# voxelmorph/voxelmorph

Measured on NVIDIA H100. Metric: vol-pairs/sec (3D 160x192x224 VxmDense int_steps=7 train step, NCC+Grad, Adam), higher is better.
Workload: dtype bf16 (conv operands) / f32 (accumulate, warp, VecInt, losses)

## Files before the change

voxelmorph_b200/csrc/conv3d_tc_s.cu:

```cuda
#include <stdlib.h>
#include <string.h>

#include "tc_common.cuh"

namespace vxm {
namespace tcs {

using namespace vxm::tc;

constexpr int WT = 32, WUSE = 30;
constexpr int MAXSLOT = 16;
constexpr int NLOADER = 128, NTHREADS = 384, NGRP = 2;

struct ConvSArgs {
  const __nv_bfloat16* xa; const __nv_bfloat16* xb;
  const __nv_bfloat16* wpk; const float* bias;
  void* out; const __nv_bfloat16* mask;
  void* out2; int csplit;
  int B, D, H, W, Ca, Cb, up, upd, Cout, out_mode;
  float slope;
  int tiles_h, tiles_w, dchunk, nchunks, nitems, nslot;
  uint32_t wbytes;
  const float* acc_in; void* out_lo;
  int tma_mask, tc0[2];
  int opitch;
  alignas(64) CUtensorMap tm[2];
};

__host__ __device__ inline uint32_t swz(uint32_t off, uint32_t width) {
  return off ^ (((off >> 7) & (width / 16 - 1)) << 4);
}
__device__ __forceinline__ uint64_t make_desc_kmajor_swz(uint32_t saddr, uint32_t width) {
  uint64_t d = 0;
  d |= (uint64_t)((saddr >> 4) & 0x3FFF);
  d |= (uint64_t)1 << 16;
  d |= (uint64_t)(((8u * width) >> 4) & 0x3FFF) << 32;
  return d | desc_swizzle(width);
}

template <int KD, int G0, int G1, int COUT, int HT, bool ACC, int EPI, bool OP = false, int PD = 0>
__global__ void __launch_bounds__(NTHREADS, 1) conv_tcs_kernel(const __grid_constant__ ConvSArgs a) {
  static_assert(PD == 0 || (KD == 3 && EPI != 0 && !ACC && !OP), "polyphase forms: 3-D, specialised epilogue");
  static_assert(PD != 1 || G1 > 0, "the polyphase forward merges channel group 0 and keeps group 1");
  static_assert(PD != 2 || (G1 == 0 && COUT == 32 && HT == 8 && EPI == 2), "the coarse dgrad: 32 -> 32 channels, 8-row tiles");
  constexpr int SROWS = (HT + 2) * WT;
  constexpr int NH = PD == 2 ? 1 : HT / 4;
  constexpr int NEVEN = (HT + 3) / 2;
  constexpr int W0 = G0 * 2, W1 = G1 * 2;
  constexpr int NC8 = (G0 + G1) / 8;
  constexpr uint32_t SLAB0 = SROWS * W0, SLAB1 = SROWS * W1;
  constexpr int NN = 3 * COUT;
  extern __shared__ __align__(1024) uint8_t smem[];
  const bool halfk = (a.Ca + a.Cb == 8);
  constexpr uint32_t slab_bytes = SLAB0 + SLAB1;
  const int NSLOT = a.nslot;
  uint8_t* s_w = smem;
  uint8_t* s_slab = smem + ((a.wbytes + 1023u) & ~1023u);
  float* s_stage = reinterpret_cast<float*>(s_slab + NSLOT * slab_bytes);
  uint64_t* bars = reinterpret_cast<uint64_t*>(s_stage + NGRP * ACC_STAGE_FLOATS);
  uint64_t* full = bars;
  uint64_t* empty = bars + MAXSLOT;
  uint64_t* wbar = empty + MAXSLOT;

  const int warp = threadIdx.x >> 5, lane = threadIdx.x & 31;

  const bool tma0 = a.tma_mask & 1, tma1 = (a.tma_mask & 2) != 0;
  const bool all_tma = tma0 && (G1 == 0 || tma1);
  if (threadIdx.x == 0) {
    for (int i = 0; i < NSLOT; ++i) { mbar_init(&full[i], all_tma ? 1 : NLOADER); mbar_init(&empty[i], 4 * NGRP); }
    mbar_init(wbar, 1);
    fence_barrier_init();
  }
  __syncthreads();

  if (threadIdx.x == 0) {
    mbar_expect_tx(wbar, a.wbytes);
    for (uint32_t off = 0; off < a.wbytes; off += 16384u) {
      uint32_t n = a.wbytes - off < 16384u ? a.wbytes - off : 16384u;
      bulk_g2s(s_w + off, reinterpret_cast<const uint8_t*>(a.wpk) + off, n, wbar);
    }
  }
  const int HW_tiles = a.tiles_h * a.tiles_w;
  const int Dout = PD == 2 ? a.D >> 1 : a.D;

  if (warp >= 8) {
    const int lt = threadIdx.x - 8 * 32;
    uint32_t slot = 0, lphase = 1;
    const int Da = a.upd ? a.D >> 1 : a.D, Ha = a.up ? a.H >> 1 : a.H, Wa = a.up ? a.W >> 1 : a.W;
    const int nca8 = a.Ca >> 3;
    constexpr int nchunk = NC8 * SROWS;
    constexpr int KMAX = (nchunk + NLOADER - 1) / NLOADER;
    if (lt == 0) {
      if (tma0) tma_prefetch_desc(&a.tm[0]);
      if (tma1) tma_prefetch_desc(&a.tm[1]);
    }
    const uint32_t tma_bytes = (tma0 ? SLAB0 : 0u) + (tma1 ? SLAB1 : 0u);
    for (int item = blockIdx.x; item < a.nitems && !(all_tma && lt != 0); item += gridDim.x) {
      const int wt = item % a.tiles_w, ht = (item / a.tiles_w) % a.tiles_h;
      const int ch = (item / HW_tiles) % a.nchunks, b = item / (HW_tiles * a.nchunks);
      const int h0 = ht * HT, w0 = wt * WUSE, d0 = ch * a.dchunk, d1 = min(d0 + a.dchunk, Dout);
      const int s_begin = PD == 2 ? 2 * d0 - 1 : (KD == 3 ? d0 - 1 : d0), s_end = PD == 2 ? 2 * d1 + 1 : (KD == 3 ? d1 + 1 : d1);
      int soff[KMAX];
      uint32_t doff[KMAX];
#pragma unroll
      for (int k = 0; k < KMAX; ++k) {
        const int id = lt + k * NLOADER;
        soff[k] = -1;
        doff[k] = 0;
        if (id < nchunk) {
          const int c8 = id % NC8, row = id / NC8;
          const int r = row >> 5, c = row & 31;
          const int h = h0 - 1 + r, w = w0 - 1 + c;
          const int srow = PD == 2 ? ((r & 1) ? NEVEN + (r >> 1) : (r >> 1)) * WT + c : row;
          doff[k] = c8 < G0 / 8 ? swz((uint32_t)srow * W0 + (uint32_t)c8 * 16u, W0)
                                : SLAB0 + swz((uint32_t)row * W1 + (uint32_t)(c8 - G0 / 8) * 16u, W1 ? W1 : 32);
          if (c8 < G0 / 8 ? tma0 : tma1) soff[k] = -2;
          else if (h >= 0 && h < a.H && w >= 0 && w < a.W && !(halfk && c8 > 0)) {
            if (c8 < nca8) soff[k] = (((a.up ? h >> 1 : h) * Wa + (a.up ? w >> 1 : w)) * a.Ca + c8 * 8) << 1;
            else soff[k] = (((h * a.W + w) * a.Cb + (c8 - nca8) * 8) << 1) | 1;
          }
        }
      }
      for (int ds = s_begin; ds < s_end; ++ds) {
        mbar_wait(&empty[slot], lphase);
        uint8_t* slab = s_slab + (size_t)slot * slab_bytes;
        const bool dok = ds >= 0 && ds < a.D;
        const __nv_bfloat16* baseA = a.xa ? a.xa + (((size_t)b * Da + (dok ? (a.upd ? ds >> 1 : ds) : 0)) * Ha * Wa) * a.Ca : nullptr;
        const __nv_bfloat16* baseB = a.xb ? a.xb + (((size_t)b * a.D + (dok ? ds : 0)) * a.H * a.W) * a.Cb : nullptr;
        const __nv_bfloat16* dummy = a.xa ? a.xa : a.xb;
        if (lt == 0 && tma_bytes) {
          if (all_tma) mbar_expect_tx(&full[slot], tma_bytes);
          else mbar_expect_tx_noarrive(&full[slot], tma_bytes);
          if (tma0) tma_load_5d(slab, &a.tm[0], a.tc0[0], w0 - 1, h0 - 1, ds, b, &full[slot]);
          if (tma1) tma_load_5d(slab + SLAB0, &a.tm[1], a.tc0[1], w0 - 1, h0 - 1, ds, b, &full[slot]);
        }
        if (!all_tma) {
#pragma unroll
          for (int k = 0; k < KMAX; ++k) {
            if (lt + k * NLOADER < nchunk && soff[k] != -2) {
              const bool ok = dok && soff[k] >= 0;
              const __nv_bfloat16* src = ok ? ((soff[k] & 1) ? baseB : baseA) + (soff[k] >> 1) : dummy;
              cp_async16(slab + doff[k], src, ok ? 16u : 0u);
            }
          }
          cp_async_arrive_noinc(&full[slot]);
        }
        if (++slot == (uint32_t)NSLOT) { slot = 0; lphase ^= 1; }
      }
    }
  } else {
    const int grp = warp >> 2;
    const int wq = warp & 3;
    float* stage = s_stage + grp * ACC_STAGE_FLOATS;
    const int nbar = 1 + grp;
    constexpr int NSUB = NN > 96 ? 2 : 1;
    constexpr int NF = 2 / NSUB;
    constexpr int NCH = NSUB == 1 ? COUT / 16 : (COUT + 31) / 32;
    const int trow0 = NSUB == 1 ? wq : (wq & 1);
    auto chan = [&](int i) { return NSUB == 1 ? 16 * i : 32 * i + 16 * (wq >> 1); };
    const uint32_t slab_u32 = smem_u32(s_slab), w_u32 = smem_u32(s_w);
    constexpr uint32_t WSTEP = (uint32_t)NN * (W0 + W1);
    mbar_wait(wbar, 0);
    const uint64_t bdesc0 = make_desc_kmajor_swz(w_u32, W0);
    const uint64_t bdesc1 = make_desc_kmajor_swz(w_u32 + NN * W0, W1 ? W1 : 32);
    uint32_t cnt_base = 0, ecnt = 0, wcur = 0;
    auto observe = [&](uint32_t upto) {
      for (; wcur <= upto; ++wcur) mbar_wait(&full[wcur % NSLOT], (wcur / NSLOT) & 1);
    };
    constexpr int NKD = PD == 2 ? 4 : KD;
    auto mma = [&](uint32_t hslot, int hb, int sub, float (&acc)[NF][NN / 2], int par) {
      uint64_t adesc0_kd[NKD], adesc1_kd[NKD];
      uint32_t sl = hslot;
#pragma unroll
      for (int kd = 0; kd < NKD; ++kd) {
        adesc0_kd[kd] = make_desc_kmajor_swz(slab_u32 + sl * slab_bytes, W0);
        adesc1_kd[kd] = make_desc_kmajor_swz(slab_u32 + sl * slab_bytes + SLAB0, W1 ? W1 : 32);
        if (++sl == (uint32_t)NSLOT) sl = 0;
      }
      wg_fence();
#pragma unroll
      for (int kd = 0; kd < NKD; ++kd) {
#pragma unroll
        for (int kh = 0; kh < (PD == 2 ? 4 : 3); ++kh) {
          const int st = kd * (PD == 2 ? 4 : 3) + kh;
#pragma unroll
          for (int k = 0; k < (G0 + G1) / 16; ++k) {
            const bool g0 = k < G0 / 16;
            if (PD == 1 && g0 && kd == 2) continue;
            const int kk = g0 ? k : k - G0 / 16;
            const uint32_t wr = g0 ? W0 : W1;
            uint64_t abase = g0 ? adesc0_kd[kd] : adesc1_kd[kd];
            uint32_t wst = st * WSTEP;
            if (PD == 1 && g0 && par) {
              abase = adesc0_kd[kd + 1 < NKD ? kd + 1 : kd];
              wst = kd == 0 ? 9 * WSTEP + kh * NN * W0 : (6 + kh) * WSTEP;
            }
            const int r0 = PD == 2 ? ((kh & 1) ? NEVEN : 0) + (kh >> 1) : hb * 4 + kh;
            const uint64_t adesc = abase + (uint64_t)((r0 * WT * wr + kk * 32) >> 4);
            const uint64_t bdesc = (g0 ? bdesc0 : bdesc1) + (uint64_t)((wst + kk * 32) >> 4);
#pragma unroll
            for (int f = 0; f < NF; ++f)
              Wgmma<NN, 0, 0>::mma(acc[f], adesc + (uint64_t)(((sub + f) * 2 * WT * wr) >> 4), bdesc, (st | k) ? 1u : 0u);
          }
        }
      }
      wg_commit();
      wg_wait<0>();
    };
    auto readout = [&](float (&acc)[NF][NN / 2], int c, uint32_t (&r)[16]) {
      if constexpr (NSUB == 1) acc_row16(acc[0], acc[NF - 1], c, stage, nbar, r);
      else acc_half_row16(acc[0], c, COUT - (c % COUT) < 32 ? 16 : 32, stage, nbar, r);
    };
    auto combine = [&](float (&acc)[NF][NN / 2], int i, float (&v)[16]) {
      const int cb = NSUB == 1 ? 16 * i : 32 * i;
      uint32_t r[16];
      readout(acc, cb, r);
#pragma unroll
      for (int c = 0; c < 16; ++c) v[c] = __shfl_up_sync(0xffffffffu, __uint_as_float(r[c]), 1);
      readout(acc, COUT + cb, r);
#pragma unroll
      for (int c = 0; c < 16; ++c) v[c] += __uint_as_float(r[c]);
      readout(acc, 2 * COUT + cb, r);
#pragma unroll
      for (int c = 0; c < 16; ++c) v[c] += __shfl_down_sync(0xffffffffu, __uint_as_float(r[c]), 1);
    };
    auto release = [&](int nd) {
      if (KD == 3) {
        const uint32_t last = PD == 2 ? 2u * nd : (uint32_t)nd;
        observe(cnt_base + last + 1u);
        if (lane == 0) {
          mbar_arrive(&empty[(cnt_base + last) % NSLOT]);
          mbar_arrive(&empty[(cnt_base + last + 1) % NSLOT]);
        }
        cnt_base += last + 2;
      } else {
        cnt_base += nd;
      }
    };
    if constexpr (EPI != 0) {
      const float slope = a.slope;
      const int c1 = (EPI == 3 && a.out2) ? a.csplit : COUT;
      const int Ho = PD == 2 ? a.H >> 1 : a.H, Wo = PD == 2 ? a.W >> 1 : a.W;
      const size_t HWp = (size_t)Ho * Wo;
      for (int item = blockIdx.x; item < a.nitems; item += gridDim.x) {
        const int wt = item % a.tiles_w, ht = (item / a.tiles_w) % a.tiles_h;
        const int ch = (item / HW_tiles) % a.nchunks, b = item / (HW_tiles * a.nchunks);
        const int w = wt * WUSE - 1 + lane, d0 = ch * a.dchunk, d1 = min(d0 + a.dchunk, Dout);
        const int nd = d1 - d0;
        const bool wok = lane >= 1 && lane <= WUSE && w < a.W && (PD != 2 || (lane & 1));
        bool ok[NH][NSUB];
        size_t vx[NH][NSUB];
#pragma unroll
        for (int hb = 0; hb < NH; ++hb) {
#pragma unroll
          for (int sub = 0; sub < NSUB; ++sub) {
            const int h = PD == 2 ? ht * (HT / 2) + trow0 : ht * HT + hb * 4 + trow0 + 2 * sub;
            ok[hb][sub] = wok && h < Ho;
            vx[hb][sub] = (((size_t)b * Dout + d0) * Ho + h) * Wo + (PD == 2 ? w >> 1 : w);
          }
        }
        for (int j = 0; j < nd; ++j) {
          const uint32_t js = PD == 2 ? 2u * j : (uint32_t)j;
          observe(cnt_base + js + (PD == 2 ? 3u : (KD == 3 ? 2u : 0u)));
          const uint32_t hslot = (cnt_base + js) % NSLOT;
#pragma unroll
          for (int hb = 0; hb < NH; ++hb) {
            const bool mine = (int)(ecnt++ % NGRP) == grp;
            size_t voxs[NSUB];
#pragma unroll
            for (int sub = 0; sub < NSUB; ++sub) {
              voxs[sub] = vx[hb][sub];
              vx[hb][sub] += HWp;
            }
            if (!mine) continue;
#pragma unroll
            for (int sub = 0; sub < NSUB; ++sub) {
              const size_t vox = voxs[sub];
              const bool valid = ok[hb][sub];
              [[maybe_unused]] uint32_t mreg[EPI == 2 ? NCH : 1][8];
              if constexpr (EPI == 2) {
#pragma unroll
                for (int i = 0; i < NCH; ++i)
                  if (valid && chan(i) < COUT) ld_global_nc_v8(a.mask + vox * (OP ? a.opitch : COUT) + chan(i), mreg[i]);
              }
              float acc[NF][NN / 2];
              mma(hslot, hb, sub, acc, (d0 + j) & 1);
#pragma unroll
              for (int i = 0; i < NCH; ++i) {
                const int c0 = chan(i);
                float v[16];
                combine(acc, i, v);
                if (NSUB > 1 && c0 >= COUT) continue;
                if constexpr (PD == 2) {
#pragma unroll
                  for (int c = 0; c < 16; ++c) v[c] += __shfl_down_sync(0xffffffffu, v[c], 1);
                }
                if constexpr (EPI == 1) {
#pragma unroll
                  for (int c = 0; c < 16; ++c) {
                    const float x = v[c] + (a.bias ? __ldg(a.bias + c0 + c) : 0.f);
                    v[c] = fmaxf(x, x * slope);
                  }
                } else if constexpr (EPI == 2) {
#pragma unroll
                  for (int e = 0; e < 8; ++e) {
                    const uint32_t mw = mreg[i][e];
                    if (mw & 0x8000u) v[2 * e] *= slope;
                    if (mw & 0x80000000u) v[2 * e + 1] *= slope;
                  }
                }
                if (valid) {
                  __nv_bfloat16* dst = (EPI == 3 && c0 >= c1) ? reinterpret_cast<__nv_bfloat16*>(a.out2) + vox * (COUT - c1) + (c0 - c1)
                                                              : reinterpret_cast<__nv_bfloat16*>(a.out) + vox * (OP ? a.opitch : c1) + c0;
                  st_global_v8(dst, pack_bf16x2(v[0], v[1]), pack_bf16x2(v[2], v[3]), pack_bf16x2(v[4], v[5]), pack_bf16x2(v[6], v[7]),
                               pack_bf16x2(v[8], v[9]), pack_bf16x2(v[10], v[11]), pack_bf16x2(v[12], v[13]), pack_bf16x2(v[14], v[15]));
                }
              }
            }
          }
          if (lane == 0) {
            mbar_arrive(&empty[hslot]);
            if (PD == 2) mbar_arrive(&empty[(hslot + 1) % NSLOT]);
          }
        }
        release(nd);
      }
    } else {
    const size_t HWp = (size_t)a.H * a.W;
    auto bias_at = [&](int c) -> float { return a.bias ? __ldg(a.bias + c) : 0.f; };
    for (int item = blockIdx.x; item < a.nitems; item += gridDim.x) {
      const int wt = item % a.tiles_w, ht = (item / a.tiles_w) % a.tiles_h;
      const int ch = (item / HW_tiles) % a.nchunks, b = item / (HW_tiles * a.nchunks);
      const int w = wt * WUSE - 1 + lane, d0 = ch * a.dchunk, d1 = min(d0 + a.dchunk, a.D);
      const int nd = d1 - d0;
      for (int j = 0; j < nd; ++j) {
        const int d = d0 + j;
        observe(cnt_base + (uint32_t)j + (KD == 3 ? 2u : 0u));
        const uint32_t hslot = (cnt_base + j) % NSLOT;
#pragma unroll
        for (int hb = 0; hb < NH; ++hb) {
        if ((int)(ecnt++ % NGRP) != grp) continue;
#pragma unroll
        for (int sub = 0; sub < NSUB; ++sub) {
        const int h = ht * HT + hb * 4 + trow0 + 2 * sub;
        const bool valid = lane >= 1 && lane <= WUSE && h < a.H && w < a.W;
        const size_t vox = (((size_t)b * a.D + d) * a.H + h) * a.W + w;
        constexpr bool PREF = NSUB == 1;
        [[maybe_unused]] uint4 mreg[PREF ? NCH : 1][2];
        if (PREF && a.mask && valid) {
#pragma unroll
          for (int i = 0; i < NCH; ++i)
#pragma unroll
            for (int q = 0; q < 2; ++q)
              if (chan(i) + 8 * q < a.Cout)
                mreg[i][q] = __ldg(reinterpret_cast<const uint4*>(a.mask + vox * (OP ? a.opitch : a.Cout) + chan(i)) + q);
        }
        const int c1 = a.out2 ? a.csplit : a.Cout;
        float acc[NF][NN / 2];
        mma(hslot, hb, sub, acc, 0);
#pragma unroll
        for (int i = 0; i < NCH; ++i) {
          const int c0 = chan(i);
          [[maybe_unused]] float4 ain[ACC ? 4 : 1];
          if constexpr (ACC && !OP && PREF) {
            if (a.acc_in && valid && c0 < COUT) {
              const float4* ap = reinterpret_cast<const float4*>(a.acc_in + vox * COUT + c0);
#pragma unroll
              for (int q = 0; q < 4; ++q) ain[q] = __ldg(ap + q);
            }
          }
          float v[16];
          combine(acc, i, v);
          if (NSUB > 1 && c0 >= COUT) continue;
          bool handled = false;
          if constexpr (ACC) {
            if (a.acc_in && valid) {
              if constexpr (OP || !PREF) {
                const float4* ap = reinterpret_cast<const float4*>(a.acc_in + vox * COUT + c0);
#pragma unroll
                for (int q = 0; q < 4; ++q) ain[q] = __ldg(ap + q);
              }
#pragma unroll
              for (int q = 0; q < 4; ++q) { v[4 * q] += ain[q].x; v[4 * q + 1] += ain[q].y; v[4 * q + 2] += ain[q].z; v[4 * q + 3] += ain[q].w; }
            }
            if (a.out_mode == 2) {
              handled = true;
              if (valid) {
                float4* op = reinterpret_cast<float4*>(reinterpret_cast<float*>(a.out) + vox * COUT + c0);
#pragma unroll
                for (int q = 0; q < 4; ++q) op[q] = make_float4(v[4 * q], v[4 * q + 1], v[4 * q + 2], v[4 * q + 3]);
              }
            } else if (a.out_mode == 3) {
              handled = true;
              if (valid && c0 < a.Cout) {
#pragma unroll
                for (int q = 0; q < 16; q += 8) {
                  if (c0 + q < a.Cout) {
                    uint32_t hi[4], lo[4];
#pragma unroll
                    for (int e = 0; e < 8; e += 2) {
                      float x0 = v[q + e] + bias_at(c0 + q + e), x1 = v[q + e + 1] + bias_at(c0 + q + e + 1);
                      if (a.slope >= 0.f) { x0 = x0 >= 0.f ? x0 : x0 * a.slope; x1 = x1 >= 0.f ? x1 : x1 * a.slope; }
                      const __nv_bfloat16 h0 = __float2bfloat16_rn(x0), h1 = __float2bfloat16_rn(x1);
                      hi[e >> 1] = (uint32_t)__bfloat16_as_ushort(h0) | ((uint32_t)__bfloat16_as_ushort(h1) << 16);
                      lo[e >> 1] = pack_bf16x2(x0 - __bfloat162float(h0), x1 - __bfloat162float(h1));
                    }
                    const size_t o = vox * (OP ? a.opitch : a.Cout) + c0 + q;
                    *reinterpret_cast<uint4*>(reinterpret_cast<__nv_bfloat16*>(a.out) + o) = make_uint4(hi[0], hi[1], hi[2], hi[3]);
                    *reinterpret_cast<uint4*>(reinterpret_cast<__nv_bfloat16*>(a.out_lo) + o) = make_uint4(lo[0], lo[1], lo[2], lo[3]);
                  }
                }
              }
            }
          }
          if (!handled && valid && c0 < a.Cout) {
            if (a.out_mode == 0) {
#pragma unroll
              for (int q = 0; q < 16; q += 8) {
                if (c0 + q < a.Cout) {
                  float x[8];
#pragma unroll
                  for (int e = 0; e < 8; ++e) x[e] = v[q + e] + bias_at(c0 + q + e);
                  if (a.mask) {
                    uint4 m4;
                    if constexpr (PREF) m4 = mreg[i][q / 8];
                    else m4 = __ldg(reinterpret_cast<const uint4*>(a.mask + vox * (OP ? a.opitch : a.Cout) + c0) + q / 8);
                    const __nv_bfloat16* mb = reinterpret_cast<const __nv_bfloat16*>(&m4);
#pragma unroll
                    for (int e = 0; e < 8; ++e) if (__bfloat162float(mb[e]) < 0.f) x[e] *= a.slope;
                  } else if (a.slope >= 0.f) {
#pragma unroll
                    for (int e = 0; e < 8; ++e) x[e] = x[e] >= 0.f ? x[e] : x[e] * a.slope;
                  }
                  const int cg = c0 + q;
                  __nv_bfloat16* oo = cg < c1 ? reinterpret_cast<__nv_bfloat16*>(a.out) + vox * (OP ? a.opitch : c1) + cg
                                              : reinterpret_cast<__nv_bfloat16*>(a.out2) + vox * (a.Cout - c1) + (cg - c1);
                  *reinterpret_cast<uint4*>(oo) = make_uint4(pack_bf16x2(x[0], x[1]), pack_bf16x2(x[2], x[3]), pack_bf16x2(x[4], x[5]), pack_bf16x2(x[6], x[7]));
                }
              }
            } else {
              float* o = reinterpret_cast<float*>(a.out);
#pragma unroll
              for (int c = 0; c < 16; ++c) {
                if (c0 + c < a.Cout) {
                  float x = v[c] + bias_at(c0 + c);
                  if (a.slope >= 0.f) x = x >= 0.f ? x : x * a.slope;
                  o[(((size_t)b * a.Cout + c0 + c) * a.D + d) * HWp + (size_t)h * a.W + w] = x;
                }
              }
            }
          }
        }
        }
        }
        if (lane == 0) mbar_arrive(&empty[hslot]);
      }
      release(nd);
    }
    }
  }
}

__global__ void pack_weights_s_kernel(const float* __restrict__ w, __nv_bfloat16* __restrict__ out, int Cout, int Cin, int KD, int COUT,
                                      int NN, int G0, int G1, int transposed) {
  const int T = KD * 9;
  const int CG = G0 + G1;
  const int total = KD * 3 * NN * CG;
  for (int i = blockIdx.x * blockDim.x + threadIdx.x; i < total; i += gridDim.x * blockDim.x) {
    const int ci = i % CG, n = (i / CG) % NN, st = i / (CG * NN);
    const int kd = st / 3, kh = st % 3, g = n / COUT, co = n % COUT;
    const int tap = (kd * 3 + kh) * 3 + g;
    float v = 0.f;
    if (!transposed) {
      if (co < Cout && ci < Cin) v = w[((size_t)co * Cin + ci) * T + tap];
    } else {
      if (co < Cin && ci < Cout) v = w[((size_t)ci * Cin + co) * T + (T - 1 - tap)];
    }
    const uint32_t W0 = G0 * 2, W1 = G1 * 2;
    uint32_t off;
    if (ci < G0) off = swz((uint32_t)n * W0 + (uint32_t)ci * 2u, W0);
    else off = (uint32_t)NN * W0 + swz((uint32_t)n * W1 + (uint32_t)(ci - G0) * 2u, W1);
    out[((size_t)st * NN * (W0 + W1) + off) / 2] = __float2bfloat16_rn(v);
  }
}

struct PackDesc {
  const float* w;
  __nv_bfloat16* out;
  int Cout, Cin, KD, COUT, NN, G0, G1, transposed;
  int begin, count;
  int fold;
  int n0, nb, k0, kb;
  int poly;
};
__global__ void pack_weights_multi_kernel(const PackDesc* __restrict__ descs, int ndesc, int total) {
  for (int gi = blockIdx.x * blockDim.x + threadIdx.x; gi < total; gi += gridDim.x * blockDim.x) {
    int lo = 0, hi = ndesc - 1;
    while (lo < hi) {
      const int mid = (lo + hi + 1) >> 1;
      if (descs[mid].begin <= gi) lo = mid; else hi = mid - 1;
    }
    const PackDesc d = descs[lo];
    const int i = gi - d.begin;
    const int T = d.KD * 9, CG = d.G0 + d.G1;
    const int base = d.KD * 3 * d.NN * CG;
    const bool extra = d.poly == 1 && i >= base;
    const int ie = i - base;
    const int ci = extra ? ie % d.G0 : i % CG, n = extra ? (ie / d.G0) % d.NN : (i / CG) % d.NN;
    const int st = extra ? ie / (d.G0 * d.NN) : i / (CG * d.NN);
    const int kd = extra ? 0 : (d.poly == 2 ? st >> 2 : st / 3), kh = extra ? st : (d.poly == 2 ? st & 3 : st % 3);
    const int g = n / d.COUT, co = n % d.COUT;
    const int tap = (kd * 3 + kh) * 3 + g;
    float v = 0.f;
    if (d.poly) {
      if (co < d.nb && ci < d.kb) {
        int t0 = kd, t1 = kd, u0 = kh, u1 = kh;
        if (d.poly == 1 && ci < d.G0) t1 = extra ? 1 : (kd == 1 ? 2 : kd);
        if (d.poly == 2) {
          t0 = kd > 0 ? kd - 1 : 0; t1 = kd < 2 ? kd : 2;
          u0 = kh > 0 ? kh - 1 : 0; u1 = kh < 2 ? kh : 2;
        }
        for (int t = t0; t <= t1; ++t)
          for (int u = u0; u <= u1; ++u) {
            const int tp = (t * 3 + u) * 3 + g;
            v += !d.transposed ? d.w[((size_t)(d.n0 + co) * d.Cin + d.k0 + ci) * 27 + tp]
                               : d.w[((size_t)(d.k0 + ci) * d.Cin + d.n0 + co) * 27 + (26 - tp)];
          }
      }
    } else if (d.fold) {
      const int fk = ci / d.fold, c = ci % d.fold;
      const int tap3 = (fk * 3 + kh) * 3 + g;
      if (fk < 3) {
        if (!d.transposed) { if (co < d.Cout) v = d.w[((size_t)co * d.Cin + c) * 27 + tap3]; }
        else if (co < d.Cin) v = d.w[((size_t)c * d.Cin + co) * 27 + (26 - tap3)];
      }
    } else if (co < d.nb && ci < d.kb) {
      if (!d.transposed) v = d.w[((size_t)(d.n0 + co) * d.Cin + d.k0 + ci) * T + tap];
      else v = d.w[((size_t)(d.k0 + ci) * d.Cin + d.n0 + co) * T + (T - 1 - tap)];
    }
    const uint32_t W0 = d.G0 * 2, W1 = d.G1 * 2;
    uint32_t off;
    if (extra) off = (uint32_t)base * 2u + (uint32_t)(st * d.NN) * W0 + swz((uint32_t)n * W0 + (uint32_t)ci * 2u, W0);
    else if (ci < d.G0) off = (uint32_t)(st * d.NN) * (W0 + W1) + swz((uint32_t)n * W0 + (uint32_t)ci * 2u, W0);
    else off = (uint32_t)(st * d.NN) * (W0 + W1) + (uint32_t)d.NN * W0 + swz((uint32_t)n * W1 + (uint32_t)(ci - d.G0) * 2u, W1);
    d.out[off / 2] = __float2bfloat16_rn(v);
  }
}

static void groups_of(int cin, int* g0, int* g1) {
  if (cin == 8 || cin == 16) { *g0 = 16; *g1 = 0; }
  else if (cin == 32) { *g0 = 32; *g1 = 0; }
  else if (cin == 48) { *g0 = 32; *g1 = 16; }
  else { *g0 = 64; *g1 = 0; }
}

static int plan_tma(ConvSArgs& a, int g0, int g1, int HTv) {
  a.tma_mask = 0;
  a.tc0[0] = a.tc0[1] = 0;
  const char* e = getenv("VXM_B200_TMA");
  if (e && e[0] == '0') return 0;
  const int lo[2] = {0, g0}, hi[2] = {g0, g0 + g1};
  for (int g = 0; g < 2; ++g) {
    if (hi[g] == lo[g]) continue;
    const void* base = nullptr;
    int C = 0, c0 = 0;
    if (a.xa && hi[g] <= a.Ca && !a.up) { base = a.xa; C = a.Ca; c0 = lo[g]; }
    else if (a.xb && lo[g] >= a.Ca && hi[g] <= a.Ca + a.Cb) { base = a.xb; C = a.Cb; c0 = lo[g] - a.Ca; }
    if (!base) continue;
    if (tc::make_act_tmap(&a.tm[g], base, a.B, a.D, a.H, a.W, C, hi[g] - lo[g], WT, HTv + 2) != 0) return -1;
    a.tma_mask |= 1 << g;
    a.tc0[g] = c0;
  }
  return 0;
}

}
}

using namespace vxm;
using namespace vxm::tcs;

extern "C" size_t vxm_conv3d_tcs_packed_bytes(int cin_eff, int coutp, int kd) {
  int g0, g1;
  groups_of(cin_eff <= 8 ? 8 : (cin_eff <= 16 ? 16 : (cin_eff <= 32 ? 32 : (cin_eff <= 48 ? 48 : 64))), &g0, &g1);
  return (size_t)kd * 3 * (3 * coutp) * (g0 + g1) * sizeof(__nv_bfloat16);
}

extern "C" int vxm_conv3d_tcs_pack(const float* w, void* wpk, int Cout, int Cin, int kd, int coutp, int transposed, void* stream) {
  VXM_REQUIRE(w && wpk && Cout > 0 && Cin > 0 && (kd == 1 || kd == 3) && (coutp == 16 || coutp == 32 || coutp == 48 || coutp == 64), "conv3d_tcs_pack: bad argument");
  int cin_eff = transposed ? Cout : Cin, nout = transposed ? Cin : Cout;
  VXM_REQUIRE(nout <= coutp, "conv3d_tcs_pack: %d output channels do not fit %d", nout, coutp);
  VXM_REQUIRE(cin_eff <= 64, "conv3d_tcs_pack: at most 64 input channels");
  int g0, g1;
  groups_of(cin_eff <= 8 ? 8 : (cin_eff <= 16 ? 16 : (cin_eff <= 32 ? 32 : (cin_eff <= 48 ? 48 : 64))), &g0, &g1);
  int NN = 3 * coutp;
  int total = kd * 3 * NN * (g0 + g1);
  pack_weights_s_kernel<<<(total + 255) / 256, 256, 0, as_stream(stream)>>>(w, (__nv_bfloat16*)wpk, Cout, Cin, kd, coutp, NN, g0, g1, transposed);
  return check_launch("conv3d_tcs_pack");
}

extern "C" size_t vxm_conv3d_tcs_pack_desc_bytes(void) { return sizeof(PackDesc); }

extern "C" int vxm_conv3d_tcs_pack_desc_blk(void* desc_host, const float* w, void* wpk, int Cout, int Cin, int kd, int coutp, int transposed,
                                            int n0, int nb, int k0, int kb, int begin) {
  VXM_REQUIRE(desc_host && w && wpk && Cout > 0 && Cin > 0 && (kd == 1 || kd == 3) && (coutp == 16 || coutp == 32 || coutp == 48 || coutp == 64),
              "conv3d_tcs_pack_desc: bad argument");
  const int cin_eff = transposed ? Cout : Cin, nout = transposed ? Cin : Cout;
  VXM_REQUIRE(n0 >= 0 && nb > 0 && n0 + nb <= nout && k0 >= 0 && kb > 0 && k0 + kb <= cin_eff, "conv3d_tcs_pack_desc: block out of range");
  VXM_REQUIRE(nb <= coutp && kb <= 64, "conv3d_tcs_pack_desc: channel counts do not fit");
  int g0, g1;
  groups_of(kb <= 8 ? 8 : (kb <= 16 ? 16 : (kb <= 32 ? 32 : (kb <= 48 ? 48 : 64))), &g0, &g1);
  PackDesc d;
  d.w = w; d.out = (__nv_bfloat16*)wpk; d.Cout = Cout; d.Cin = Cin; d.KD = kd; d.COUT = coutp; d.NN = 3 * coutp; d.G0 = g0; d.G1 = g1;
  d.transposed = transposed; d.begin = begin; d.count = kd * 3 * d.NN * (g0 + g1); d.fold = 0;
  d.n0 = n0; d.nb = nb; d.k0 = k0; d.kb = kb; d.poly = 0;
  memcpy(desc_host, &d, sizeof(d));
  return d.count;
}

extern "C" int vxm_conv3d_tcs_pack_desc(void* desc_host, const float* w, void* wpk, int Cout, int Cin, int kd, int coutp, int transposed,
                                        int begin) {
  VXM_REQUIRE(Cout > 0 && Cin > 0, "conv3d_tcs_pack_desc: bad argument");
  return vxm_conv3d_tcs_pack_desc_blk(desc_host, w, wpk, Cout, Cin, kd, coutp, transposed, 0, transposed ? Cin : Cout, 0,
                                      transposed ? Cout : Cin, begin);
}

extern "C" int vxm_conv3d_tcs_pack_desc_fold(void* desc_host, const float* w, void* wpk, int Cout, int Cin, int coutp, int transposed, int begin) {
  VXM_REQUIRE(desc_host && w && wpk && Cout > 0 && Cin > 0 && (coutp == 16 || coutp == 32), "conv3d_tcs_pack_desc_fold: bad argument");
  const int real_in = transposed ? Cout : Cin, nout = transposed ? Cin : Cout;
  VXM_REQUIRE(3 * real_in <= 16 && nout <= coutp, "conv3d_tcs_pack_desc_fold: %d x 3 input channels / %d outputs do not fit", real_in, nout);
  int g0, g1;
  groups_of(3 * real_in <= 8 ? 8 : 16, &g0, &g1);
  PackDesc d;
  d.w = w; d.out = (__nv_bfloat16*)wpk; d.Cout = Cout; d.Cin = Cin; d.KD = 1; d.COUT = coutp; d.NN = 3 * coutp; d.G0 = g0; d.G1 = g1;
  d.transposed = transposed; d.begin = begin; d.count = 3 * d.NN * (g0 + g1); d.fold = real_in;
  d.n0 = d.nb = d.k0 = d.kb = 0; d.poly = 0;
  memcpy(desc_host, &d, sizeof(d));
  return d.count;
}

static int poly_geometry(int mode, int Cout, int Cin, int Ca, int* g0, int* g1, int* kd, int* coutp) {
  if (mode == 1 && Ca == 32 && Cin == 48 && Cout == 32) { *g0 = 32; *g1 = 16; *kd = 3; *coutp = 32; return 1; }
  if (mode == 2 && Ca == 32 && Cin > Ca && Cout == 32) { *g0 = 32; *g1 = 0; *kd = 4; *coutp = 32; return 1; }
  return 0;
}

static size_t poly_bytes(int mode) {
  const size_t NN = 3 * 32;
  return (mode == 1 ? 9 * NN * (32 + 16) + 3 * NN * 32 : 16 * NN * 32) * sizeof(__nv_bfloat16);
}

extern "C" size_t vxm_conv3d_tcs_poly_packed_bytes(int mode, int Cout, int Cin, int Ca) {
  int g0, g1, kd, coutp;
  return poly_geometry(mode, Cout, Cin, Ca, &g0, &g1, &kd, &coutp) ? poly_bytes(mode) : 0;
}

extern "C" int vxm_conv3d_tcs_pack_desc_poly(void* desc_host, const float* w, void* wpk, int Cout, int Cin, int Ca, int mode, int begin) {
  int g0, g1, kd, coutp;
  VXM_REQUIRE(desc_host && w && wpk && poly_geometry(mode, Cout, Cin, Ca, &g0, &g1, &kd, &coutp),
              "conv3d_tcs_pack_desc_poly: no polyphase operand for mode %d, (%d of %d) -> %d", mode, Ca, Cin, Cout);
  PackDesc d;
  d.w = w; d.out = (__nv_bfloat16*)wpk; d.Cout = Cout; d.Cin = Cin; d.KD = kd; d.COUT = coutp; d.NN = 3 * coutp; d.G0 = g0; d.G1 = g1;
  d.transposed = mode == 2; d.begin = begin; d.fold = 0; d.poly = mode;
  d.n0 = 0; d.nb = mode == 1 ? Cout : Ca; d.k0 = 0; d.kb = mode == 1 ? Cin : Cout;
  d.count = (int)(vxm_conv3d_tcs_poly_packed_bytes(mode, Cout, Cin, Ca) / sizeof(__nv_bfloat16));
  memcpy(desc_host, &d, sizeof(d));
  return d.count;
}

extern "C" int vxm_conv3d_tcs_pack_multi(const void* descs_dev, int ndesc, int total, void* stream) {
  VXM_REQUIRE(descs_dev && ndesc > 0 && total > 0, "conv3d_tcs_pack_multi: bad argument");
  const int blocks = (total + 255) / 256, cap = sm_count() * 8;
  pack_weights_multi_kernel<<<blocks < cap ? blocks : cap, 256, 0, as_stream(stream)>>>((const PackDesc*)descs_dev, ndesc, total);
  return check_launch("conv3d_tcs_pack_multi");
}

extern "C" int vxm_conv3d_tcs_supported(int Ca, int Cb, int Cout) {
  int cin = Ca + Cb;
  bool split_ok = cin != 48 || (Ca == 32 && Cb == 16) || Cb == 0 || Ca == 0;
  return (Cout <= 64) && (cin == 8 || cin == 16 || cin == 32 || cin == 48 || cin == 64) && Ca % 8 == 0 && Cb % 8 == 0 && split_ok;
}

static int conv_tcs_launch(const void* xa, const void* xb, const void* wpk, const float* bias, void* out, const void* mask,
                           int B, int D, int H, int W, int Ca, int Cb, int up, int Cout, int coutp, int kd, int out_mode,
                           float slope, void* out2, int csplit, const float* acc_in, void* out_lo, int opitch, int poly,
                           void* stream);

extern "C" int vxm_conv3d_tcs_poly(const void* xa, const void* xb, const void* wpk, const float* bias, void* out, const void* mask, int B,
                                   int D, int H, int W, int Ca, int Cb, int Cout, int mode, float slope, void* stream) {
  VXM_REQUIRE(mode == 1 || mode == 2, "conv3d_tcs_poly: mode must be 1 (forward) or 2 (coarse dgrad)");
  return conv_tcs_launch(xa, xb, wpk, bias, out, mask, B, D, H, W, Ca, Cb, mode == 1 ? 1 : 0, Cout, 32, 3, 0, slope, nullptr, 0,
                         nullptr, nullptr, 0, mode, stream);
}

static size_t fixed_smem(uint32_t wbytes) { return ((wbytes + 1023u) & ~1023u) + NGRP * ACC_STAGE_FLOATS * sizeof(float) + 1024 + 512; }

extern "C" int vxm_conv3d_tcs_fits(int cin, int coutp, int kd) {
  int g0, g1;
  groups_of(cin <= 8 ? 8 : (cin <= 16 ? 16 : (cin <= 32 ? 32 : (cin <= 48 ? 48 : 64))), &g0, &g1);
  const size_t slab4 = (size_t)6 * WT * (g0 + g1) * 2;
  return fixed_smem((uint32_t)vxm_conv3d_tcs_packed_bytes(cin, coutp, kd)) + 4 * slab4 <= 227 * 1024;
}

extern "C" int vxm_conv3d_tcs_fwd(const void* xa, const void* xb, const void* wpk, const float* bias, void* out, const void* mask,
                                  int B, int D, int H, int W, int Ca, int Cb, int up, int Cout, int coutp, int kd, int out_mode,
                                  float slope, void* out2, int csplit, void* stream) {
  VXM_REQUIRE(out_mode == 0 || out_mode == 1, "conv3d_tcs_fwd: out_mode must be 0 (bf16 channels-last) or 1 (fp32 planar)");
  return conv_tcs_launch(xa, xb, wpk, bias, out, mask, B, D, H, W, Ca, Cb, up, Cout, coutp, kd, out_mode, slope, out2, csplit,
                         nullptr, nullptr, 0, 0, stream);
}

extern "C" int vxm_conv3d_tcs_fwd_blk(const void* xa, const void* xb, const void* wpk, const float* bias, void* out, void* out_lo,
                                      const void* mask, const float* acc_in, int B, int D, int H, int W, int Ca, int Cb, int up, int Cout,
                                      int coutp, int kd, int out_mode, float slope, int opitch, void* stream) {
  VXM_REQUIRE(out_mode == 0 || out_mode == 2 || out_mode == 3, "conv3d_tcs_fwd_blk: out_mode must be 0 (bf16), 2 (fp32 partial sums) or 3 (bf16 hi/lo pair)");
  VXM_REQUIRE(out_mode != 3 || out_lo, "conv3d_tcs_fwd_blk: out_mode 3 needs out_lo");
  VXM_REQUIRE(opitch == 0 || (opitch >= Cout && opitch % 8 == 0 && out_mode != 2), "conv3d_tcs_fwd_blk: bad output pitch %d", opitch);
  return conv_tcs_launch(xa, xb, wpk, bias, out, mask, B, D, H, W, Ca, Cb, up, Cout, coutp, kd, out_mode, slope, nullptr, 0,
                         acc_in, out_lo, opitch == Cout ? 0 : opitch, 0, stream);
}

extern "C" int vxm_conv3d_tcs2_fwd(const void* xa, const void* xb, const void* wpk, const float* bias, void* out, const void* mask,
                                   int B, int D, int H, int W, int Ca, int Cb, int up, int Cout, int coutp, int kd, int out_mode,
                                   float slope, void* out2, int csplit, void* stream) {
  return vxm_conv3d_tcs_fwd(xa, xb, wpk, bias, out, mask, B, D, H, W, Ca, Cb, up, Cout, coutp, kd, out_mode, slope, out2, csplit, stream);
}

extern "C" int vxm_conv3d_tcs_fwd_acc(const void* xa, const void* xb, const void* wpk, const float* bias, void* out, void* out_lo,
                                      const float* acc_in, int B, int D, int H, int W, int Ca, int Cb, int up, int Cout, int coutp,
                                      int kd, int out_mode, float slope, void* stream) {
  VXM_REQUIRE(out_mode >= 1 && out_mode <= 3, "conv3d_tcs_fwd_acc: out_mode must be 1 (fp32 planar), 2 (fp32 partial sums) or 3 (bf16 hi/lo pair)");
  VXM_REQUIRE(out_mode != 3 || out_lo, "conv3d_tcs_fwd_acc: out_mode 3 needs out_lo");
  return conv_tcs_launch(xa, xb, wpk, bias, out, nullptr, B, D, H, W, Ca, Cb, up, Cout, coutp, kd, out_mode, slope, nullptr, 0,
                         acc_in, out_lo, 0, 0, stream);
}

static int conv_tcs_launch(const void* xa, const void* xb, const void* wpk, const float* bias, void* out, const void* mask,
                           int B, int D, int H, int W, int Ca, int Cb, int up, int Cout, int coutp, int kd, int out_mode,
                           float slope, void* out2, int csplit, const float* acc_in, void* out_lo, int opitch, int poly,
                           void* stream) {
  VXM_REQUIRE(B > 0 && D > 0 && H > 0 && W > 0 && wpk && out, "conv3d_tcs_fwd: bad argument");
  VXM_REQUIRE(kd == 1 || kd == 3, "conv3d_tcs_fwd: kd must be 1 or 3");
  VXM_REQUIRE(coutp == 16 || coutp == 32 || coutp == 48 || coutp == 64, "conv3d_tcs_fwd: padded Cout must be 16, 32, 48 or 64");
  VXM_REQUIRE(!out2 || (out_mode == 0 && csplit > 0 && csplit < Cout && csplit % 8 == 0 && !mask), "conv3d_tcs_fwd: bad output split");
  VXM_REQUIRE(Cout > 0 && Cout <= coutp && (out_mode == 1 || out_mode == 2 || Cout % 8 == 0), "conv3d_tcs_fwd: unsupported Cout %d", Cout);
  VXM_REQUIRE(vxm_conv3d_tcs_supported(Ca, Cb, Cout), "conv3d_tcs_fwd: channel counts (%d,%d)->%d unsupported", Ca, Cb, Cout);
  VXM_REQUIRE((Ca == 0 || xa) && (Cb == 0 || xb), "conv3d_tcs_fwd: missing source tensor");
  VXM_REQUIRE(!up || (H % 2 == 0 && W % 2 == 0 && (kd == 1 || D % 2 == 0)), "conv3d_tcs_fwd: upsampled source needs even sizes");
  VXM_REQUIRE(poly == 0 || (kd == 3 && coutp == 32 && Cout == 32 && out_mode == 0 && !out2 && !acc_in && !opitch &&
                            (poly == 1 ? up && Ca == 32 && Cb == 16 && bias && !mask && slope >= 0.f && slope <= 1.f
                                       : !up && Ca == 32 && Cb == 0 && !bias && mask && D % 2 == 0 && H % 2 == 0 && W % 2 == 0)),
              "conv3d_tcs_poly: no polyphase mode %d kernel for (%d,%d)->%d", poly, Ca, Cb, Cout);
  ConvSArgs a{};
  const int cin = Ca + Cb;
  int g0, g1;
  groups_of(cin, &g0, &g1);
  a.xa = (const __nv_bfloat16*)xa; a.xb = (const __nv_bfloat16*)xb; a.wpk = (const __nv_bfloat16*)wpk; a.bias = bias;
  a.out = out; a.mask = (const __nv_bfloat16*)mask; a.out2 = out2; a.csplit = csplit;
  a.acc_in = acc_in; a.out_lo = out_lo;
  a.B = B; a.D = D; a.H = H; a.W = W; a.Ca = Ca; a.Cb = Cb; a.up = up; a.upd = (up && kd == 3) ? 1 : 0;
  a.Cout = Cout; a.out_mode = out_mode; a.slope = slope; a.opitch = opitch;
  VXM_REQUIRE(!opitch || (!out2 && out_mode != 1 && kd == 3 && coutp == 32 && ((g0 == 64 && g1 == 0) || (g0 == 32 && g1 == 16))),
              "conv3d_tcs_fwd: no blocked kernel for (%d,%d)->%d/%d, kd %d", Ca, Cb, Cout, coutp, kd);
  a.wbytes = (uint32_t)(poly ? poly_bytes(poly) : vxm_conv3d_tcs_packed_bytes(cin, coutp, kd));
  const size_t fixed = fixed_smem(a.wbytes);
  int HTv = 4;
  {
    const size_t slab8 = (size_t)10 * WT * (g0 + g1) * 2;
    const int ns8 = (int)((227 * 1024 - fixed) / slab8);
    const char* e = getenv("VXM_B200_TCS_HT");
    if (g0 <= 32 && coutp <= 32 && ns8 >= (kd == 3 ? 5 : 3) && H > 4 && !(e && e[0] == '4') && !opitch) HTv = 8;
    if (poly) HTv = poly == 2 ? 8 : 4;
  }
  a.tiles_h = (H + HTv - 1) / HTv; a.tiles_w = (W + WUSE - 1) / WUSE;
  int nsm = conv_ctas();
  const long long tiles = (long long)B * a.tiles_h * a.tiles_w;
  int best_nch = 1;
  double best_cost = 1e300;
  const int Do = poly == 2 ? D / 2 : D;
  for (int nch = 1; nch <= 40 && nch <= Do; ++nch) {
    const int dc = (Do + nch - 1) / nch;
    const long long items = tiles * ((Do + dc - 1) / dc);
    const long long waves = (items + nsm - 1) / nsm;
    const double cost = (double)waves * (dc + (poly == 2 ? 1.25 : (kd == 3 ? 2.5 : 0.5)));
    if (cost < best_cost - 1e-9) { best_cost = cost; best_nch = nch; }
  }
  a.dchunk = (Do + best_nch - 1) / best_nch; a.nchunks = (Do + a.dchunk - 1) / a.dchunk;
  a.nitems = (int)(tiles * a.nchunks);
  const size_t slab = (size_t)(HTv + 2) * WT * (g0 + g1) * 2;
  int nslot = (int)((227 * 1024 - fixed) / slab);
  {
    const char* e = getenv("VXM_B200_RING");
    const int cap = e ? atoi(e) : MAXSLOT;
    if (nslot > cap) nslot = cap;
    if (nslot > MAXSLOT) nslot = MAXSLOT;
  }
  VXM_REQUIRE(nslot >= 4, "conv3d_tcs_fwd: not enough shared memory for the slab ring");
  a.nslot = nslot;
  size_t smem = fixed + (size_t)nslot * slab;
  int grid = a.nitems < nsm ? a.nitems : nsm;
  cudaStream_t st = as_stream(stream);
  if (poly != 2 && plan_tma(a, g0, g1, HTv) != 0) return VXM_ERR_CUDA;
  const bool acc_epi = acc_in != nullptr || out_mode >= 2;
  int epi = 0;
  {
    const char* e = getenv("VXM_B200_TCS_EPI");
    const bool plain = kd == 3 && out_mode == 0 && !acc_epi && Cout == coutp && !(e && e[0] == '0');
    if (plain && !out2 && !mask && slope >= 0.f && slope <= 1.f) epi = 1;
    else if (plain && !out2 && mask && !bias) epi = 2;
    else if (plain && !mask && !bias && slope < 0.f && (!out2 || csplit % 16 == 0)) epi = 3;
    if (poly) epi = poly;
  }
#define VXM_TCS_LAUNCH_E(KD_, G0_, G1_, CO_, HT_, ACC_, E_, ...)                                                                  \
  do {                                                                                                                            \
    VXM_CUDA(cudaFuncSetAttribute(conv_tcs_kernel<KD_, G0_, G1_, CO_, HT_, ACC_, E_, ##__VA_ARGS__>,                              \
                                  cudaFuncAttributeMaxDynamicSharedMemorySize, (int)smem));                                       \
    conv_tcs_kernel<KD_, G0_, G1_, CO_, HT_, ACC_, E_, ##__VA_ARGS__><<<grid, NTHREADS, smem, st>>>(a);                           \
  } while (0)
#define VXM_TCS_LAUNCH_OP(G0_, G1_)                                                                                               \
  do {                                                                                                                            \
    if (acc_epi) VXM_TCS_LAUNCH_E(3, G0_, G1_, 32, 4, true, 0, true);                                                             \
    else if (epi == 1) VXM_TCS_LAUNCH_E(3, G0_, G1_, 32, 4, false, 1, true);                                                      \
    else if (epi == 2) VXM_TCS_LAUNCH_E(3, G0_, G1_, 32, 4, false, 2, true);                                                      \
    else if (epi == 3) VXM_TCS_LAUNCH_E(3, G0_, G1_, 32, 4, false, 3, true);                                                      \
    else VXM_TCS_LAUNCH_E(3, G0_, G1_, 32, 4, false, 0, true);                                                                    \
  } while (0)
#define VXM_TCS_LAUNCH(KD_, G0_, G1_, CO_, HT_)                                                                                   \
  do {                                                                                                                            \
    if (acc_epi) VXM_TCS_LAUNCH_E(KD_, G0_, G1_, CO_, HT_, true, 0);                                                              \
    else if (KD_ == 3 && epi == 1) VXM_TCS_LAUNCH_E(3, G0_, G1_, CO_, HT_, false, 1);                                             \
    else if (KD_ == 3 && epi == 2) VXM_TCS_LAUNCH_E(3, G0_, G1_, CO_, HT_, false, 2);                                             \
    else if (KD_ == 3 && epi == 3) VXM_TCS_LAUNCH_E(3, G0_, G1_, CO_, HT_, false, 3);                                             \
    else VXM_TCS_LAUNCH_E(KD_, G0_, G1_, CO_, HT_, false, 0);                                                                     \
  } while (0)
#define VXM_TCS_G8(KD_, CO_)                                                  \
  do {                                                                        \
    if (g0 == 16) VXM_TCS_LAUNCH(KD_, 16, 0, CO_, 8);                         \
    else if (g0 == 32 && g1 == 0) VXM_TCS_LAUNCH(KD_, 32, 0, CO_, 8);         \
    else VXM_TCS_LAUNCH(KD_, 32, 16, CO_, 8);                                 \
  } while (0)
#define VXM_TCS_G(KD_, CO_)                                                   \
  do {                                                                        \
    if (g0 == 16) VXM_TCS_LAUNCH(KD_, 16, 0, CO_, 4);                         \
    else if (g0 == 32 && g1 == 0) VXM_TCS_LAUNCH(KD_, 32, 0, CO_, 4);         \
    else if (g0 == 32) VXM_TCS_LAUNCH(KD_, 32, 16, CO_, 4);                   \
    else VXM_TCS_LAUNCH(KD_, 64, 0, CO_, 4);                                  \
  } while (0)
  if (poly) {
    if (poly == 1) VXM_TCS_LAUNCH_E(3, 32, 16, 32, 4, false, 1, false, 1);
    else VXM_TCS_LAUNCH_E(3, 32, 0, 32, 8, false, 2, false, 2);
  } else if (opitch) {
    if (g0 == 64) VXM_TCS_LAUNCH_OP(64, 0); else VXM_TCS_LAUNCH_OP(32, 16);
  } else if (HTv == 8) {
    if (kd == 3) { if (coutp == 16) VXM_TCS_G8(3, 16); else VXM_TCS_G8(3, 32); }
    else { if (coutp == 16) VXM_TCS_G8(1, 16); else VXM_TCS_G8(1, 32); }
  } else if (kd == 3) { if (coutp == 16) VXM_TCS_G(3, 16); else if (coutp == 32) VXM_TCS_G(3, 32); else if (coutp == 48) VXM_TCS_G(3, 48); else VXM_TCS_G(3, 64); }
  else { if (coutp == 16) VXM_TCS_G(1, 16); else if (coutp == 32) VXM_TCS_G(1, 32); else if (coutp == 48) VXM_TCS_G(1, 48); else VXM_TCS_G(1, 64); }
  return check_launch("conv3d_tcs_fwd");
}
```

Measured before the change: 69.57.

## Write conv epilogue directly from MMA fragment layout with seam exchange via shared memory

For the non-row epilogue path, the per-voxel combine of accumulator fragments is replaced. Partial sums are now combined in place through warp shuffles, and the tile-seam values are exchanged between warp pairs through the shared stage buffer under a named barrier. Each lane then stores bf16x2 values straight from the fragment layout and loads mask words to match. The intent is to avoid the full 16-channel combine and reduce register and shuffle traffic, at the cost of an extra barrier, narrower 4-byte stores, and more complex validity masking.

```diff
diff --git a/voxelmorph_b200/csrc/conv3d_tc_s.cu b/voxelmorph_b200/csrc/conv3d_tc_s.cu
--- a/voxelmorph_b200/csrc/conv3d_tc_s.cu
+++ b/voxelmorph_b200/csrc/conv3d_tc_s.cu
@@ -242,82 +242,172 @@
       const int c1 = (EPI == 3 && a.out2) ? a.csplit : COUT;
       const int Ho = PD == 2 ? a.H >> 1 : a.H, Wo = PD == 2 ? a.W >> 1 : a.W;
       const size_t HWp = (size_t)Ho * Wo;
+      const int q = lane >> 2, p = lane & 3, half = wq & 1, pair = wq >> 1;
+      const int xbar = 3 + 2 * grp + pair;
+      constexpr bool ROWS = NSUB > 1 || PD == 2;
+      constexpr int XPAIR = NF * 2 * COUT;
+      static_assert(2 * 2 * XPAIR <= ACC_STAGE_FLOATS, "seam exchange fits the stage buffer");
+      uint32_t xpar = 0;
       for (int item = blockIdx.x; item < a.nitems; item += gridDim.x) {
         const int wt = item % a.tiles_w, ht = (item / a.tiles_w) % a.tiles_h;
         const int ch = (item / HW_tiles) % a.nchunks, b = item / (HW_tiles * a.nchunks);
-        const int w = wt * WUSE - 1 + lane, d0 = ch * a.dchunk, d1 = min(d0 + a.dchunk, Dout);
+        const int d0 = ch * a.dchunk, d1 = min(d0 + a.dchunk, Dout);
         const int nd = d1 - d0;
-        const bool wok = lane >= 1 && lane <= WUSE && w < a.W && (PD != 2 || (lane & 1));
-        bool ok[NH][NSUB];
-        size_t vx[NH][NSUB];
-#pragma unroll
-        for (int hb = 0; hb < NH; ++hb) {
-#pragma unroll
-          for (int sub = 0; sub < NSUB; ++sub) {
-            const int h = PD == 2 ? ht * (HT / 2) + trow0 : ht * HT + hb * 4 + trow0 + 2 * sub;
-            ok[hb][sub] = wok && h < Ho;
-            vx[hb][sub] = (((size_t)b * Dout + d0) * Ho + h) * Wo + (PD == 2 ? w >> 1 : w);
-          }
-        }
+        const int wp = 16 * half + q, w = wt * WUSE - 1 + wp;
+        const int hbase = ht * HT + pair;
+        uint32_t okm = 0;
+#pragma unroll
+        for (int hb = 0; hb < NH; ++hb)
+#pragma unroll
+          for (int blk = 0; blk < 2; ++blk)
+#pragma unroll
+            for (int i = 0; i < 2; ++i)
+              if (wp + 8 * i >= 1 && wp + 8 * i <= WUSE && w + 8 * i < a.W && hbase + 4 * hb + 2 * blk < Ho)
+                okm |= 1u << (4 * hb + 2 * blk + i);
+        size_t vbase = (((size_t)b * Dout + d0) * Ho + hbase) * Wo + (size_t)(long long)w;
         for (int j = 0; j < nd; ++j) {
           const uint32_t js = PD == 2 ? 2u * j : (uint32_t)j;
           observe(cnt_base + js + (PD == 2 ? 3u : (KD == 3 ? 2u : 0u)));
           const uint32_t hslot = (cnt_base + js) % NSLOT;
 #pragma unroll
           for (int hb = 0; hb < NH; ++hb) {
-            const bool mine = (int)(ecnt++ % NGRP) == grp;
-            size_t voxs[NSUB];
+            if ((int)(ecnt++ % NGRP) != grp) continue;
+            auto vox_of = [&](int blk, int i) { return vbase + (size_t)((4 * hb + 2 * blk) * Wo + 8 * i); };
 #pragma unroll
             for (int sub = 0; sub < NSUB; ++sub) {
-              voxs[sub] = vx[hb][sub];
-              vx[hb][sub] += HWp;
-            }
-            if (!mine) continue;
-#pragma unroll
-            for (int sub = 0; sub < NSUB; ++sub) {
-              const size_t vox = voxs[sub];
-              const bool valid = ok[hb][sub];
-              [[maybe_unused]] uint32_t mreg[EPI == 2 ? NCH : 1][8];
-              if constexpr (EPI == 2) {
+              [[maybe_unused]] uint32_t mreg[EPI == 2 && !ROWS ? NF : 1][2][COUT / 8];
+              auto load_mask = [&](int f) {
+                if constexpr (EPI == 2 && !ROWS) {
+#pragma unroll
+                  for (int i = 0; i < 2; ++i)
+                    if (okm >> (4 * hb + 2 * f + i) & 1u) {
+                      const uint32_t* mp = reinterpret_cast<const uint32_t*>(a.mask + vox_of(f, i) * (OP ? a.opitch : COUT) + 2 * p);
+#pragma unroll
+                      for (int jj = 0; jj < COUT / 8; ++jj) mreg[f][i][jj] = __ldg(mp + 4 * jj);
+                    }
+                }
+              };
+              if constexpr (COUT == 16) {
+#pragma unroll
+                for (int f = 0; f < NF; ++f) load_mask(f);
+              }
+              const int rh = PD == 2 ? ht * (HT / 2) + trow0 : ht * HT + hb * 4 + trow0 + 2 * sub, rw = wt * WUSE - 1 + lane;
+              const bool rvalid = lane >= 1 && lane <= WUSE && rw < a.W && rh < Ho && (PD != 2 || (lane & 1));
+              const size_t rvox = (((size_t)b * Dout + d0 + j) * Ho + rh) * Wo + (PD == 2 ? rw >> 1 : rw);
+              [[maybe_unused]] uint32_t mrow[PD == 2 ? NCH : 1][8];
+              if constexpr (PD == 2) {
 #pragma unroll
                 for (int i = 0; i < NCH; ++i)
-                  if (valid && chan(i) < COUT) ld_global_nc_v8(a.mask + vox * (OP ? a.opitch : COUT) + chan(i), mreg[i]);
+                  if (rvalid) ld_global_nc_v8(a.mask + rvox * COUT + chan(i), mrow[i]);
               }
               float acc[NF][NN / 2];
               mma(hslot, hb, sub, acc, (d0 + j) & 1);
-#pragma unroll
-              for (int i = 0; i < NCH; ++i) {
-                const int c0 = chan(i);
-                float v[16];
-                combine(acc, i, v);
-                if (NSUB > 1 && c0 >= COUT) continue;
-                if constexpr (PD == 2) {
-#pragma unroll
-                  for (int c = 0; c < 16; ++c) v[c] += __shfl_down_sync(0xffffffffu, v[c], 1);
-                }
-                if constexpr (EPI == 1) {
-#pragma unroll
-                  for (int c = 0; c < 16; ++c) {
-                    const float x = v[c] + (a.bias ? __ldg(a.bias + c0 + c) : 0.f);
-                    v[c] = fmaxf(x, x * slope);
+              if constexpr (ROWS) {
+                const bool valid = rvalid;
+                const size_t vox = rvox;
+#pragma unroll
+                for (int i = 0; i < NCH; ++i) {
+                  const int c0 = chan(i);
+                  float v[16];
+                  combine(acc, i, v);
+                  if (c0 >= COUT) continue;
+                  if constexpr (PD == 2) {
+#pragma unroll
+                    for (int c = 0; c < 16; ++c) v[c] += __shfl_down_sync(0xffffffffu, v[c], 1);
                   }
-                } else if constexpr (EPI == 2) {
-#pragma unroll
-                  for (int e = 0; e < 8; ++e) {
-                    const uint32_t mw = mreg[i][e];
-                    if (mw & 0x8000u) v[2 * e] *= slope;
-                    if (mw & 0x80000000u) v[2 * e + 1] *= slope;
+                  if constexpr (EPI == 1) {
+#pragma unroll
+                    for (int c = 0; c < 16; ++c) {
+                      const float x = v[c] + (a.bias ? __ldg(a.bias + c0 + c) : 0.f);
+                      v[c] = fmaxf(x, x * slope);
+                    }
+                  } else if constexpr (EPI == 2) {
+                    uint32_t mreg[8];
+                    if constexpr (PD == 2) {
+#pragma unroll
+                      for (int e = 0; e < 8; ++e) mreg[e] = mrow[i][e];
+                    } else if (valid) {
+                      ld_global_nc_v8(a.mask + vox * (OP ? a.opitch : COUT) + c0, mreg);
+                    }
+#pragma unroll
+                    for (int e = 0; e < 8; ++e) {
+                      if (mreg[e] & 0x8000u) v[2 * e] *= slope;
+                      if (mreg[e] & 0x80000000u) v[2 * e + 1] *= slope;
+                    }
+                  }
+                  if (valid) {
+                    __nv_bfloat16* dst = (EPI == 3 && c0 >= c1) ? reinterpret_cast<__nv_bfloat16*>(a.out2) + vox * (COUT - c1) + (c0 - c1)
+                                                                : reinterpret_cast<__nv_bfloat16*>(a.out) + vox * (OP ? a.opitch : c1) + c0;
+                    st_global_v8(dst, pack_bf16x2(v[0], v[1]), pack_bf16x2(v[2], v[3]), pack_bf16x2(v[4], v[5]), pack_bf16x2(v[6], v[7]),
+                                 pack_bf16x2(v[8], v[9]), pack_bf16x2(v[10], v[11]), pack_bf16x2(v[12], v[13]), pack_bf16x2(v[14], v[15]));
                   }
                 }
-                if (valid) {
-                  __nv_bfloat16* dst = (EPI == 3 && c0 >= c1) ? reinterpret_cast<__nv_bfloat16*>(a.out2) + vox * (COUT - c1) + (c0 - c1)
-                                                              : reinterpret_cast<__nv_bfloat16*>(a.out) + vox * (OP ? a.opitch : c1) + c0;
-                  st_global_v8(dst, pack_bf16x2(v[0], v[1]), pack_bf16x2(v[2], v[3]), pack_bf16x2(v[4], v[5]), pack_bf16x2(v[6], v[7]),
-                               pack_bf16x2(v[8], v[9]), pack_bf16x2(v[10], v[11]), pack_bf16x2(v[12], v[13]), pack_bf16x2(v[14], v[15]));
+                continue;
+              }
+              float* xb = stage + xpar * (2 * XPAIR) + pair * XPAIR;
+              xpar ^= 1u;
+              if (half == 0 ? q == 7 : q == 0) {
+#pragma unroll
+                for (int f = 0; f < NF; ++f)
+#pragma unroll
+                  for (int jj = 0; jj < COUT / 8; ++jj) {
+                    float2* xs = reinterpret_cast<float2*>(xb + f * 2 * COUT + 8 * jj + 2 * p);
+                    const int k0 = 4 * jj + 2, k2 = 4 * (COUT / 4 + jj);
+                    if (half == 0) xs[0] = make_float2(acc[f][k0], acc[f][k0 + 1]);
+                    else xs[COUT / 2] = make_float2(acc[f][k2], acc[f][k2 + 1]);
+                  }
+              }
+              named_bar(xbar, 64);
+#pragma unroll
+              for (int f = 0; f < NF; ++f) {
+                const int blk = sub + f;
+                if constexpr (COUT != 16) load_mask(f);
+#pragma unroll
+                for (int jj = 0; jj < COUT / 8; ++jj) {
+                  const int c0 = 8 * jj + 2 * p;
+                  float v[2][2];
+#pragma unroll
+                  for (int e = 0; e < 2; ++e) {
+                    const float* xs = xb + f * 2 * COUT + c0 + e;
+                    const int k0 = 4 * jj + e, k1 = 4 * (COUT / 8 + jj) + e, k2 = 4 * (COUT / 4 + jj) + e;
+                    const float a1 = __shfl_sync(0xffffffffu, q == 7 ? acc[f][k0] : acc[f][k0 + 2], (lane + 28) & 31);
+                    const float a0 = __shfl_sync(0xffffffffu, acc[f][k0], (lane + 28) & 31);
+                    const float b0 = __shfl_sync(0xffffffffu, q == 0 ? acc[f][k2 + 2] : acc[f][k2], (lane + 4) & 31);
+                    const float b1 = __shfl_sync(0xffffffffu, acc[f][k2 + 2], (lane + 4) & 31);
+                    float x0 = q == 0 ? xs[0] : a0;
+                    x0 += acc[f][k1];
+                    x0 += b0;
+                    float x1 = a1;
+                    x1 += acc[f][k1 + 2];
+                    x1 += q == 7 ? xs[COUT] : b1;
+                    v[0][e] = x0;
+                    v[1][e] = x1;
+                  }
+#pragma unroll
+                  for (int i = 0; i < 2; ++i) {
+                    if constexpr (EPI == 1) {
+#pragma unroll
+                      for (int e = 0; e < 2; ++e) {
+                        const float x = v[i][e] + (a.bias ? __ldg(a.bias + c0 + e) : 0.f);
+                        v[i][e] = fmaxf(x, x * slope);
+                      }
+                    } else if constexpr (EPI == 2) {
+                      const uint32_t mw = mreg[f][i][jj];
+                      if (mw & 0x8000u) v[i][0] *= slope;
+                      if (mw & 0x80000000u) v[i][1] *= slope;
+                    }
+                    if (okm >> (4 * hb + 2 * blk + i) & 1u) {
+                      const size_t vox = vox_of(blk, i);
+                      __nv_bfloat16* dst = (EPI == 3 && c0 >= c1) ? reinterpret_cast<__nv_bfloat16*>(a.out2) + vox * (COUT - c1) + (c0 - c1)
+                                                                  : reinterpret_cast<__nv_bfloat16*>(a.out) + vox * (OP ? a.opitch : c1) + c0;
+                      *reinterpret_cast<uint32_t*>(dst) = pack_bf16x2(v[i][0], v[i][1]);
+                    }
+                  }
                 }
               }
             }
           }
+          vbase += HWp;
           if (lane == 0) {
             mbar_arrive(&empty[hslot]);
             if (PD == 2) mbar_arrive(&empty[(hslot + 1) % NSLOT]);
```

Result: faster. 76.26, median of 6 (+9.6%).
